# peterdavidfagan/mujoco_robot_environments

Measured on AMD Instinct MI355X. Metric: env steps/sec (whole node), RearrangementEnv batch=4096 at 1/2/4/8 MI355X, higher is better.
Workload: dtype f32

## Files before the change

### mujoco_robot_environments_amd/csrc/mre_dev.h

```cpp
#pragma once
#include <stdint.h>

namespace mre {

constexpr int NB = 20;
constexpr int NRB = 16;
constexpr int GRIP_BODY0 = 8;
constexpr int NV = 39;
constexpr int NRV = 15;
constexpr int NQ = 43;
constexpr int NQP = 44;
constexpr int TRACE_W = 88;
constexpr int TRACE_QVEL = 48;
constexpr int NVP = 40;
constexpr int NU = 8;
constexpr int QFINE = 32;
constexpr int QFINE_ROW = 96;
constexpr int QFINE_CUBE_Q = 32;
constexpr int QFINE_CUBE_V = 60;
static_assert(QFINE_CUBE_Q + 7 * 4 == QFINE_CUBE_V && QFINE_CUBE_V + 6 * 4 <= QFINE_ROW, "qfine row layout");
constexpr int NPROP = 4;
constexpr int NG = 20;
constexpr int PROP_GEOM0 = 12;
constexpr int NPAIR = 128;
// ... 20 lines not shown
constexpr int MAXBLK = 58;
#elif defined(MRE_LARGE_CAPS)
constexpr int NCON_MAX = 44;
constexpr int NEFC_MAX = 148;
constexpr int NRROW_MAX = 83;
constexpr int NPP_MAX = 16;
constexpr int MAXBLK = 52;
#elif defined(MRE_NEWTON)
constexpr int NCON_MAX = 32;
constexpr int NEFC_MAX = 112;
constexpr int NRROW_MAX = 69;
constexpr int NPP_MAX = 8;
constexpr int MAXBLK = 40;
#else
constexpr int NCON_MAX = 32;
constexpr int NEFC_MAX = 112;
constexpr int NRROW_MAX = 62;
constexpr int NPP_MAX = 8;
constexpr int MAXBLK = 40;
#endif
constexpr int NRROW_MAX_COMPACT_PGS = 62, NRROW_MAX_COMPACT_NEWTON = 69;
#if !defined(MRE_LARGE_CAPS)
static_assert(NRROW_MAX ==
#ifdef MRE_NEWTON
              NRROW_MAX_COMPACT_NEWTON,
#else
              NRROW_MAX_COMPACT_PGS,
#endif
              "host-side copy of the compact robot-row capacity");
#endif
static_assert(NEFC_MAX <= 256 && NRROW_MAX < 127 && NPP_MAX <= 16 && MAXBLK >= 8 + NCON_MAX,
              "capacities must fit the block descriptor fields (mre_solver.h)");

struct alignas(16) PairRec {
  int g1, g2, b1, b2;
  int pid1, pid2, type1, single;
  float pos1[3], rb1;
  float pos2[3], rb2;
  float quat1[4], quat2[4];
  float size1[3], margin;
  float size2[3], gap;
};
static_assert(sizeof(PairRec) == 128, "PairRec is eight 16-byte words");

struct alignas(16) BodyRec {
  float quat[4];
  float pos[3], mass;
  float jnt_pos[3], qpos0;
  float jnt_axis[3]; int qposadr;
  float ipos[3]; int propid;
  float iquat[4];
  float inertia[3]; int dofadr;
  float jnt_range[2], invweight0[2];
  float jnt_stiffness, jnt_springref; int parent, jnt_limited;
};
static_assert(sizeof(BodyRec) == 144, "BodyRec is nine 16-byte words");
struct alignas(16) DofRec {
  int body, propid, dofadr, ten;
  float armature, damping, invweight0, ten_coef;
  float jnt_stiffness, jnt_springref, act_gain, act_bias0;
  float act_bias1, act_bias2, act_ctrl_lo, act_ctrl_hi;
  float act_force_lo, act_force_hi; int act_forcelimited, pad;
};
static_assert(sizeof(DofRec) == 80, "DofRec is five 16-byte words");
struct alignas(16) MEntryRec {
  int i, j; float armature, damping;
  float act_bias2, ten_coef; int ten, pad;
};
static_assert(sizeof(MEntryRec) == 32, "MEntryRec is two 16-byte words");
struct alignas(16) RowRec {
  float solref[2], margin, gap;
  float solimp[5], friction;
  float invw1, invw2;
};
static_assert(sizeof(RowRec) == 48, "RowRec is three 16-byte words");
constexpr int ROWREC_JNT = NEQ, ROWREC_PAIR = NEQ + NB, NROWREC = NEQ + NB + NPAIR;
// ... 3 lines not shown
  float data[8];
  float qpos0_1, qpos0_2; int pad2, root_chain_len;
  int root_chain[12];
};
static_assert(sizeof(EqRec) == 128 && MAXCHAIN <= 12, "EqRec is eight 16-byte words");
struct alignas(16) SiteRec {
  float pos[3]; int body;
  float quat[4];
};
static_assert(sizeof(SiteRec) == 32, "SiteRec is two 16-byte words");
struct alignas(16) OptRec {
  float timestep, impratio, tolerance; int iterations;
  float gravity[3]; int cone;
  float ten_coef[2]; int ten_dof[2];
  float grip_gainprm, grip_biasprm[3];
  float grip_forcerange[2], grip_ctrlrange[2];
  float robot_mass, M0_diag_robot_sum; int tcp_site, eef_site;
  float tcp_pos[3]; int pad;
};
static_assert(sizeof(OptRec) == 112, "OptRec is seven 16-byte words");

struct DevModel {
  int body_propid[NB];
  int chain_len[NB];
  int chain_dof[NB][MAXCHAIN];
  float body_mass[NB];
  int dof_Madr[NV + 1];
  float qpos0[NQP];
  int M_i[NMR], M_j[NMR];
  int geom_type[NG], geom_body[NG], geom_propid[NG];
  float geom_size[NG][3], geom_pos[NG][3], geom_quat[NG][4], geom_rbound[NG];
  int pair_g1[NPAIR], pair_g2[NPAIR];
  float pair_margin[NPAIR];
  PairRec pair_rec[NPAIR];
  float act_ctrlrange[NU][2];
  float home_qpos[7];
  float park_pos[NPROP][3];
  BodyRec body_rec[NB];
  DofRec dof_rec[NV];
  MEntryRec m_rec[NMR];
  RowRec row_rec[NROWREC];
  EqRec eq_rec[NEQ];
  SiteRec site_rec[NSITE];
  OptRec opt_rec;
};

struct OscConfig {
  float kp_pos, kd_pos, kp_ori, kd_ori, kp_null, kd_null;
  float null_q[7];
  float pos_thresh, ori_thresh;
  int pinv_always;
};

enum StepFlags : unsigned { F_NO_CONSTRAINTS = 1u, F_FREEZE_ROBOT = 2u, F_CONV_CONTINUE = 4u, F_CONV_OPEN = 8u,
                            F_OSC_EVAL = 16u, F_DETECT = 32u, F_SETTLE_EXIT = 64u, F_DETECT_ACTIVE = 128u,
                            F_CLIP_ALWAYS = 256u, F_NW_ALL_TILES = 512u };
enum CtrlMode : int { CTRL_HELD = 0, CTRL_SEQ = 1, CTRL_OSC = 2 };

struct StepArgs {
  const DevModel* M;
  int N;
  float* qpos;
  float* qvel;
  float* qacc_ws;
  float* qfine;
  float* ctrl;
// ... 127 lines not shown
```

### mujoco_robot_environments_amd/csrc/mre_model.cpp

```cpp
#include "mre_model.h"

#include <cstdint>
#include <cstring>
#include <vector>

#include "../../include/mre.h"

namespace mre {

namespace {
struct Blob {
  const unsigned char* p;
  size_t n;
  bool find(const char* name, uint32_t* code, uint32_t* count, uint64_t* off) const {
    uint32_t ne;
    memcpy(&ne, p + 8, 4);
    const unsigned char* t = p + 16;
    for (uint32_t k = 0; k < ne; k++, t += 48)
      if (strncmp((const char*)t, name, 32) == 0) {
        memcpy(code, t + 32, 4); memcpy(count, t + 36, 4); memcpy(off, t + 40, 8);
        return *off + (size_t)(*count) * (*code ? 8 : 4) <= n;
      }
    return false;
  }
// ... 72 lines not shown
  for (int e = 0; e < NEQ; e++) {
    RowRec& r = m.row_rec[e];
    const int b1 = t.eq_obj[e][0], b2 = t.eq_obj[e][1];
    for (int c = 0; c < 2; c++) r.solref[c] = t.eq_solref[e][c];
    for (int c = 0; c < 5; c++) r.solimp[c] = t.eq_solimp[e][c];
    r.invw1 = e < 2 ? t.body_invweight0[b1][0] : t.dof_invweight0[b1 - 1];
    r.invw2 = e < 2 ? t.body_invweight0[b2][0] : t.dof_invweight0[b2 - 1];
    EqRec& q = m.eq_rec[e];
    memset(&q, 0, sizeof(q));
    q.type = t.eq_type[e]; q.b1 = b1; q.b2 = b2; q.pb1 = t.body_parent[b1]; q.pb2 = t.body_parent[b2];
    q.root = b1;
    while (q.root >= GRIP_BODY0) q.root = t.body_parent[q.root];
    for (int c = 0; c < 8; c++) q.data[c] = t.eq_data[e][c];
    q.qpos0_1 = t.qpos0[b1 - 1]; q.qpos0_2 = t.qpos0[b2 - 1];
    q.root_chain_len = t.chain_len[q.root];
    for (int c = 0; c < MAXCHAIN; c++) q.root_chain[c] = t.chain_dof[q.root][c];
  }
  for (int b = 1; b < NRB; b++) {
    RowRec& r = m.row_rec[ROWREC_JNT + b];
    for (int c = 0; c < 2; c++) r.solref[c] = t.jnt_solref[b][c];
    for (int c = 0; c < 5; c++) r.solimp[c] = t.jnt_solimp[b][c];
    r.invw1 = t.dof_invweight0[b - 1];
  }
  for (int k = 0; k < NPAIR; k++) {
    if (t.pair_g1[k] < 0) continue;
    RowRec& r = m.row_rec[ROWREC_PAIR + k];
    const int b1 = t.geom_body[t.pair_g1[k]], b2 = t.geom_body[t.pair_g2[k]];
    for (int c = 0; c < 2; c++) r.solref[c] = t.pair_solref[k][c];
    for (int c = 0; c < 5; c++) r.solimp[c] = t.pair_solimp[k][c];
    r.margin = t.pair_margin[k]; r.gap = t.pair_gap[k]; r.friction = t.pair_friction[k][0];
    r.invw1 = (b1 > 0 && b1 < NRB) ? t.body_invweight0[b1][0] : 0.f;
    r.invw2 = (b2 > 0 && b2 < NRB) ? t.body_invweight0[b2][0] : 0.f;
  }
  for (int k = 0; k < NSITE; k++) {
    SiteRec& r = m.site_rec[k];
    memset(&r, 0, sizeof(r));
    if (t.site_body[k] < 0 || t.site_body[k] >= NB) return "site_bodyid names a body that does not exist";
    r.body = t.site_body[k];
    for (int c = 0; c < 3; c++) r.pos[c] = t.site_pos[k][c];
    for (int c = 0; c < 4; c++) r.quat[c] = t.site_quat[k][c];
  }
  {
    OptRec& o = m.opt_rec;
    memset(&o, 0, sizeof(o));
    o.timestep = t.timestep; o.impratio = t.impratio; o.tolerance = t.tolerance; o.iterations = t.iterations;
    for (int c = 0; c < 3; c++) { o.gravity[c] = t.gravity[c]; o.grip_biasprm[c] = t.grip_biasprm[c]; }
    o.cone = t.cone;
    for (int c = 0; c < 2; c++) { o.ten_coef[c] = t.ten_coef[c]; o.ten_dof[c] = t.ten_dof[c]; o.grip_forcerange[c] = t.grip_forcerange[c];
                                  o.grip_ctrlrange[c] = t.act_ctrlrange[NU - 1][c]; }
    o.grip_gainprm = t.grip_gainprm; o.robot_mass = t.robot_mass; o.M0_diag_robot_sum = t.M0_diag_robot_sum;
    o.tcp_site = t.tcp_site; o.eef_site = t.eef_site;
    for (int c = 0; c < 3; c++) o.tcp_pos[c] = t.site_pos[t.tcp_site][c];
  }

  bool ok = true;
#define SAME(a, b) ok = ok && sizeof(a) == sizeof(b) && same_bits(&(a), &(b), sizeof(a))
  for (int b = 0; b < NB && ok; b++) {
    const BodyRec& r = m.body_rec[b];
    SAME(r.quat, t.body_quat[b]); SAME(r.pos, t.body_pos[b]); SAME(r.mass, t.body_mass[b]); SAME(r.jnt_pos, t.jnt_pos[b]);
    SAME(r.jnt_axis, t.jnt_axis[b]); SAME(r.qposadr, t.body_qposadr[b]); SAME(r.ipos, t.body_ipos[b]);
    SAME(r.propid, t.body_propid[b]); SAME(r.iquat, t.body_iquat[b]); SAME(r.inertia, t.body_inertia[b]);
    SAME(r.dofadr, t.body_dofadr[b]); SAME(r.jnt_range, t.jnt_range[b]); SAME(r.invweight0, t.body_invweight0[b]);
    SAME(r.jnt_stiffness, t.jnt_stiffness[b]); SAME(r.jnt_springref, t.jnt_springref[b]); SAME(r.parent, t.body_parent[b]);
    SAME(r.jnt_limited, t.jnt_limited[b]);
    if (b >= 1) SAME(r.qpos0, t.qpos0[t.body_qposadr[b]]);
  }
// ... 19 lines not shown
    SAME(r.armature, t.dof_armature[i]); SAME(r.damping, t.dof_damping[i]);
    if (i < 7) SAME(r.act_bias2, t.act_bias[i][2]);
    ok = ok && r.ten == (i == t.ten_dof[0] ? 0 : (i == t.ten_dof[1] ? 1 : -1));
    if (r.ten >= 0) SAME(r.ten_coef, t.ten_coef[r.ten]);
  }
  for (int e = 0; e < NEQ && ok; e++) {
    const RowRec& r = m.row_rec[e];
    const EqRec& q = m.eq_rec[e];
    const int b1 = t.eq_obj[e][0], b2 = t.eq_obj[e][1];
    SAME(r.solref, t.eq_solref[e]); SAME(r.solimp, t.eq_solimp[e]);
    if (e < 2) { SAME(r.invw1, t.body_invweight0[b1][0]); SAME(r.invw2, t.body_invweight0[b2][0]); }
    else { SAME(r.invw1, t.dof_invweight0[b1 - 1]); SAME(r.invw2, t.dof_invweight0[b2 - 1]); }
    SAME(q.type, t.eq_type[e]); SAME(q.b1, t.eq_obj[e][0]); SAME(q.b2, t.eq_obj[e][1]);
    SAME(q.pb1, t.body_parent[b1]); SAME(q.pb2, t.body_parent[b2]); SAME(q.data, t.eq_data[e]);
    SAME(q.qpos0_1, t.qpos0[b1 - 1]); SAME(q.qpos0_2, t.qpos0[b2 - 1]);
    int root = b1;
    while (root >= GRIP_BODY0) root = t.body_parent[root];
    ok = ok && q.root == root;
    SAME(q.root_chain_len, t.chain_len[root]);
    for (int c = 0; c < MAXCHAIN; c++) SAME(q.root_chain[c], t.chain_dof[root][c]);
  }
  for (int b = 1; b < NRB && ok; b++) {
    const RowRec& r = m.row_rec[ROWREC_JNT + b];
    SAME(r.solref, t.jnt_solref[b]); SAME(r.solimp, t.jnt_solimp[b]); SAME(r.invw1, t.dof_invweight0[b - 1]);
  }
  for (int k = 0; k < NPAIR && ok; k++) {
    if (t.pair_g1[k] < 0) continue;
    const RowRec& r = m.row_rec[ROWREC_PAIR + k];
    const int b1 = t.geom_body[t.pair_g1[k]], b2 = t.geom_body[t.pair_g2[k]];
    SAME(r.solref, t.pair_solref[k]); SAME(r.solimp, t.pair_solimp[k]); SAME(r.margin, t.pair_margin[k]);
    SAME(r.gap, t.pair_gap[k]); SAME(r.friction, t.pair_friction[k][0]);
    if (b1 > 0 && b1 < NRB) SAME(r.invw1, t.body_invweight0[b1][0]);
    if (b2 > 0 && b2 < NRB) SAME(r.invw2, t.body_invweight0[b2][0]);
  }
  for (int k = 0; k < NSITE && ok; k++) {
    const SiteRec& r = m.site_rec[k];
    SAME(r.body, t.site_body[k]); SAME(r.pos, t.site_pos[k]); SAME(r.quat, t.site_quat[k]);
  }
  {
    const OptRec& o = m.opt_rec;
    SAME(o.timestep, t.timestep); SAME(o.impratio, t.impratio); SAME(o.tolerance, t.tolerance); SAME(o.iterations, t.iterations);
    SAME(o.gravity, t.gravity); SAME(o.cone, t.cone); SAME(o.ten_coef, t.ten_coef); SAME(o.ten_dof, t.ten_dof);
    SAME(o.grip_gainprm, t.grip_gainprm); SAME(o.grip_biasprm, t.grip_biasprm); SAME(o.grip_forcerange, t.grip_forcerange);
    SAME(o.grip_ctrlrange, t.act_ctrlrange[NU - 1]); SAME(o.robot_mass, t.robot_mass);
    SAME(o.M0_diag_robot_sum, t.M0_diag_robot_sum); SAME(o.tcp_site, t.tcp_site); SAME(o.eef_site, t.eef_site);
    SAME(o.tcp_pos, t.site_pos[t.tcp_site]);
  }
#undef SAME
  if (!ok) return "a packed model record differs from the table it was filled from";
  return std::string();
}

std::string build_model(const void* blob, size_t nbytes, DevModel& m, int& solver) {
  if (nbytes < 16) return "blob too small";
  Blob b{(const unsigned char*)blob, nbytes};
  uint32_t magic;
  memcpy(&magic, b.p, 4);
  if (magic != 0x4D524542u) return "bad blob magic";
  uint32_t nentry;
  memcpy(&nentry, b.p + 8, 4);
  if (16 + 48 * (size_t)nentry > nbytes) return "blob too small";
  ModelTables t;
  memset(&t, 0, sizeof(t));
  memset(&m, 0, sizeof(m));
  int nbody, nv, nq, nM, ngeom, nsite, npair, neq, nprop, nu;
  RI("nbody", &nbody, 1); RI("nv", &nv, 1); RI("nq", &nq, 1); RI("nM", &nM, 1); RI("ngeom", &ngeom, 1);
// ... 1 lines not shown
  RI("nu", &nu, 1);
  if (nbody != NB || nv != NV || nq != NQ || ngeom != NG || nsite != NSITE || npair > NPAIR ||
      neq != NEQ || nprop != NPROP || nu != NU)
    return "scene dimensions differ from the compiled kernels";
  int body_jnttype[NB], act_dof[NU];
  RI("body_parentid", t.body_parent, NB); RI("body_jnttype", body_jnttype, NB);
  RI("body_dofadr", t.body_dofadr, NB); RI("body_qposadr", t.body_qposadr, NB);
  RI("body_propid", t.body_propid, NB);
  RF("body_pos", t.body_pos, NB * 3); RF("body_quat", t.body_quat, NB * 4);
  RF("body_ipos", t.body_ipos, NB * 3); RF("body_iquat", t.body_iquat, NB * 4);
  RF("body_mass", t.body_mass, NB); RF("body_inertia", t.body_inertia, NB * 3);
  RF("body_invweight0", t.body_invweight0, NB * 2);
  RF("jnt_pos", t.jnt_pos, NB * 3); RF("jnt_axis", t.jnt_axis, NB * 3); RF("jnt_range", t.jnt_range, NB * 2);
  RF("jnt_stiffness", t.jnt_stiffness, NB); RF("jnt_springref", t.jnt_springref, NB);
  RF("jnt_solref", t.jnt_solref, NB * 2); RF("jnt_solimp", t.jnt_solimp, NB * 5);
  RI("jnt_limited", t.jnt_limited, NB);
  RI("dof_bodyid", t.dof_body, NV); RI("dof_parentid", t.dof_parent, NV); RI("dof_Madr", t.dof_Madr, NV);
  t.dof_Madr[NV] = nM;
  RF("dof_armature", t.dof_armature, NV); RF("dof_damping", t.dof_damping, NV);
  RF("dof_invweight0", t.dof_invweight0, NV); RF("qpos0", t.qpos0, NQ);
  RI("geom_type", t.geom_type, NG); RI("geom_bodyid", t.geom_body, NG); RI("geom_propid", t.geom_propid, NG);
  RF("geom_size", t.geom_size, NG * 3); RF("geom_pos", t.geom_pos, NG * 3);
  RF("geom_quat", t.geom_quat, NG * 4); RF("geom_rbound", t.geom_rbound, NG);
  {
    std::vector<int> pg(2 * npair);
    RI("pair_geom", pg.data(), 2 * npair);
    for (int k = 0; k < NPAIR; k++) { t.pair_g1[k] = -1; t.pair_g2[k] = -1; }
    for (int k = 0; k < npair; k++) { t.pair_g1[k] = pg[2 * k]; t.pair_g2[k] = pg[2 * k + 1]; }
  }
  RI("pair_single", t.pair_single, npair);
  RF("pair_friction", t.pair_friction, npair * 3); RF("pair_solref", t.pair_solref, npair * 2);
  RF("pair_solimp", t.pair_solimp, npair * 5); RF("pair_margin", t.pair_margin, npair);
  RF("pair_gap", t.pair_gap, npair);
  for (int k = 0; k < NPAIR; k++) {
    PairRec& r = m.pair_rec[k];
    memset(&r, 0, sizeof(r));
    r.g1 = t.pair_g1[k]; r.g2 = t.pair_g2[k];
    if (r.g1 < 0) { r.g2 = -1; r.b1 = r.b2 = 0; r.pid1 = r.pid2 = -1; continue; }
    if (r.g1 >= NG || r.g2 < 0 || r.g2 >= NG) return "pair table names a geom that does not exist";
    r.b1 = t.geom_body[r.g1]; r.b2 = t.geom_body[r.g2];
    r.pid1 = t.geom_propid[r.g1]; r.pid2 = t.geom_propid[r.g2];
    r.type1 = t.geom_type[r.g1]; r.single = (t.pair_single[k] & 0xFF) | (t.geom_type[r.g2] << 8);
    if (t.geom_type[r.g1] == 2 || (t.geom_type[r.g2] == 2 && t.geom_type[r.g1] != 1))
      return "cylinder pairs: only box (geom 1) - cylinder (geom 2) is implemented";
    for (int c = 0; c < 3; c++) { r.pos1[c] = t.geom_pos[r.g1][c]; r.pos2[c] = t.geom_pos[r.g2][c];
                                  r.size1[c] = t.geom_size[r.g1][c]; r.size2[c] = t.geom_size[r.g2][c]; }
    for (int c = 0; c < 4; c++) { r.quat1[c] = t.geom_quat[r.g1][c]; r.quat2[c] = t.geom_quat[r.g2][c]; }
    r.rb1 = t.geom_rbound[r.g1]; r.rb2 = t.geom_rbound[r.g2];
    r.margin = t.pair_margin[k]; r.gap = t.pair_gap[k];
  }
  RI("site_bodyid", t.site_body, NSITE); RF("site_pos", t.site_pos, NSITE * 3);
  RF("site_quat", t.site_quat, NSITE * 4);
  RI("eef_site", &t.eef_site, 1); RI("tcp_site", &t.tcp_site, 1);
  RI("eq_type", t.eq_type, NEQ); RI("eq_obj", t.eq_obj, NEQ * 2); RF("eq_data", t.eq_data, NEQ * 8);
  RF("eq_solref", t.eq_solref, NEQ * 2); RF("eq_solimp", t.eq_solimp, NEQ * 5);
  RI("ten_dof", t.ten_dof, 2); RF("ten_coef", t.ten_coef, 2);
  RI("act_dof", act_dof, NU); RF("act_ctrlrange", t.act_ctrlrange, NU * 2);
  RF("grip_gainprm", &t.grip_gainprm, 1); RF("grip_biasprm", t.grip_biasprm, 3);
  RF("grip_forcerange", t.grip_forcerange, 2);
  for (int a = 0; a < NU; a++) { t.act_gain[a] = 1.f; t.act_forcelimited[a] = 0; }
  { uint32_t c, cnt; uint64_t off;
    if (b.find("act_gainprm", &c, &cnt, &off)) {
      RF("act_gainprm", t.act_gain, NU); RF("act_biasprm", t.act_bias, NU * 3);
      RF("act_forcerange", t.act_forcerange, NU * 2); RI("act_forcelimited", t.act_forcelimited, NU);
    } }
  RF("opt_timestep", &t.timestep, 1); RF("opt_gravity", t.gravity, 3); RF("opt_impratio", &t.impratio, 1);
  RF("opt_tolerance", &t.tolerance, 1); RI("opt_iterations", &t.iterations, 1);
  solver = MRE_SOLVER_PGS;
  { uint32_t c, cnt; uint64_t off; if (b.find("opt_solver", &c, &cnt, &off)) RI("opt_solver", &solver, 1); }
  if (solver != MRE_SOLVER_PGS && solver != MRE_SOLVER_NEWTON) return "opt_solver must be 0 (PGS) or 2 (Newton)";
  { uint32_t c, cnt; uint64_t off; int cone = 1;
    if (b.find("opt_cone", &c, &cnt, &off)) RI("opt_cone", &cone, 1);
    if (cone != 0 && cone != 1) return "opt_cone must be 0 (pyramidal) or 1 (elliptic)";
    t.cone = cone; }
  RF("home_qpos", t.home_qpos, 7);
  float M0d[NV];
  RF("M0_diag", M0d, NV);

  for (int bb = 1; bb < NB; bb++) {
    bool ok = bb < NRB ? (body_jnttype[bb] == 1 && t.body_dofadr[bb] == bb - 1 && t.body_qposadr[bb] == bb - 1 &&
                          t.body_propid[bb] < 0 && t.body_parent[bb] < bb)
                       : (body_jnttype[bb] == 2 && t.body_dofadr[bb] == NRV + 6 * (bb - NRB) &&
// ... 55 lines not shown
```

### mujoco_robot_environments_amd/csrc/mre_solver.h

```cpp
#pragma once

namespace mre {

constexpr int HDR_NONE = 0xFF;
constexpr int BLK_NONE = 0x7F;
constexpr int SCHED_NONE = 0xFF;
constexpr int TAB_OFF = MAXBLK * 5;
constexpr int TAB_ZEROS = 48;
static_assert(TAB_BYTES == 8 * (TAB_OFF + 1) + 4 * TAB_ZEROS, "operand table size");

#ifndef MRE_NEWTON
MRE_DEV void build_schedule(ModelP M, Sm& s);
#endif
MRE_DEV constexpr int cube_pair_bit(int p, int q) {
  const int a = p < q ? p : q, b = p < q ? q : p;
  return a == 0 ? b - 1 : (a == 1 ? b + 1 : 5);
}

MRE_DEV float prop_invM(const Sm& s, int p, int k) {
  return 1.0f / ((k < 3) ? s.prop_mass[p] : s.prop_inertia[p][k - 3]);
}

MRE_DEV void geom_pose(ModelP M, const Sm& s, int g, float* p, float* R, float* size,
                       float* rbound) {
  const int b = M->geom_body[g];
  float tmp[3], q[4];
  m3mulv(tmp, s.xmat[b], M->geom_pos[g]);
  v3add(p, s.xpos[b], tmp);
  qmul(q, s.xquat[b], M->geom_quat[g]);
  q2mat(R, q);
  const int pid = M->geom_propid[g];
  if (pid >= 0) {
    v3copy(size, s.prop_size[pid]);
    *rbound = v3norm(size);
  } else {
    v3copy(size, M->geom_size[g]);
    *rbound = M->geom_rbound[g];
  }
}

MRE_DEV void geom_center(ModelP M, const Sm& s, int g, float* p, float* rbound) {
  const int b = M->geom_body[g];
  float tmp[3];
  m3mulv(tmp, s.xmat[b], M->geom_pos[g]);
  v3add(p, s.xpos[b], tmp);
  const int pid = M->geom_propid[g];
  *rbound = pid >= 0 ? v3norm(s.prop_size[pid]) : M->geom_rbound[g];
}

MRE_PHASE_FN int collide_broad(ModelP M, Sm& s, int l, bool detect) {
  static_assert(offsetof(Sm, hdr) + sizeof(((Sm*)0)->hdr) - offsetof(Sm, JpA) >= sizeof(float) * 64 * COLL_BUF,
                "clip buffers do not fit");
  static_assert(NPAIR <= 256 && sizeof(((Sm*)0)->iscr) >= NPAIR, "survivor list: one byte per pair");
  MRE_DBG_T0();
  uint8_t* list = reinterpret_cast<uint8_t*>(s.iscr);
  const unsigned long long lt = (1ull << l) - 1ull;
  int nsurv = 0;
  for (int pass = 0; pass < NPAIR / 64; pass++) {
    const int pr = l + 64 * pass;
    const auto* R = &M->pair_rec[pr];
    const int g1 = R->g1, b1 = R->b1, b2 = R->b2, pid1 = R->pid1, pid2 = R->pid2, type1 = R->type1;
    const float lp1[3] = {R->pos1[0], R->pos1[1], R->pos1[2]}, lp2[3] = {R->pos2[0], R->pos2[1], R->pos2[2]};
    const float mrb1 = R->rb1, mrb2 = R->rb2, margin = R->margin, gap = R->gap;
    const float lq1[4] = {R->quat1[0], R->quat1[1], R->quat1[2], R->quat1[3]};
    bool live = false;
    if (g1 >= 0 && (pid1 < 0 || pid1 < s.nprops) && (pid2 < 0 || pid2 < s.nprops)) {
      const float inc = detect ? margin : margin - gap;
      float p1[3], p2[3], df[3], tmp[3];
      m3mulv(tmp, s.xmat[b1], lp1); v3add(p1, s.xpos[b1], tmp);
      m3mulv(tmp, s.xmat[b2], lp2); v3add(p2, s.xpos[b2], tmp);
      const float rb1 = pid1 >= 0 ? v3norm(s.prop_size[pid1]) : mrb1, rb2 = pid2 >= 0 ? v3norm(s.prop_size[pid2]) : mrb2;
      v3sub(df, p2, p1);
      if (type1 == 0) {
        float q[4], R1[9];
        qmul(q, s.xquat[b1], lq1);
        q2mat(R1, q);
        const float nn[3] = {R1[2], R1[5], R1[8]};
        live = v3dot(df, nn) - rb2 <= inc;
      } else {
        const float r = rb1 + rb2 + inc;
        live = v3dot(df, df) <= r * r;
      }
    }
    const unsigned long long m = __ballot(live);
    if (live) list[nsurv + __popcll(m & lt)] = (uint8_t)pr;
    nsurv += __popcll(m);
  }
  if (l == 0) s.ncon = 0;
  MRE_SYNC();
  MRE_DBG_STAMP(6, 0);
  return nsurv;
}
MRE_PHASE_FN int collide_narrow(ModelP M, Sm& s, int l, bool detect, bool clip_always, int c0, int nsurv, int base) {
  MRE_DBG_T0();
  float* buf = &s.JpA[0][0] + l * COLL_BUF;
  const uint8_t* list = reinterpret_cast<const uint8_t*>(s.iscr);
  const unsigned long long lt = (1ull << l) - 1ull;
  {
    const int pr = (c0 + l < nsurv) ? list[c0 + l] : -1;
    float normal[3] = {0.f, 0.f, 1.f};
    int n = 0;
    FaceCand rc;
    unsigned rm = 0u;
    if (pr >= 0) {
      const auto* R = &M->pair_rec[pr];
      const int b1 = R->b1, b2 = R->b2, pid1 = R->pid1, pid2 = R->pid2, type1 = R->type1;
      const float lp1[3] = {R->pos1[0], R->pos1[1], R->pos1[2]}, lp2[3] = {R->pos2[0], R->pos2[1], R->pos2[2]};
      const float lq1[4] = {R->quat1[0], R->quat1[1], R->quat1[2], R->quat1[3]};
      const float lq2[4] = {R->quat2[0], R->quat2[1], R->quat2[2], R->quat2[3]};
      const float ms1[3] = {R->size1[0], R->size1[1], R->size1[2]}, ms2[3] = {R->size2[0], R->size2[1], R->size2[2]};
      const float margin = R->margin, gap = R->gap;
      float p1[3], R1[9], s1[3], p2[3], R2[9], s2[3], tmp[3], q[4];
      m3mulv(tmp, s.xmat[b1], lp1); v3add(p1, s.xpos[b1], tmp);
      qmul(q, s.xquat[b1], lq1); q2mat(R1, q);
      m3mulv(tmp, s.xmat[b2], lp2); v3add(p2, s.xpos[b2], tmp);
      qmul(q, s.xquat[b2], lq2); q2mat(R2, q);
      if (pid1 >= 0) v3copy(s1, s.prop_size[pid1]); else v3copy(s1, ms1);
      if (pid2 >= 0) v3copy(s2, s.prop_size[pid2]); else v3copy(s2, ms2);
      const float inc = detect ? margin : margin - gap;
      MRE_DBG_STAMP(6, 1);
      if ((R->single >> 8) == 2) n = cyl_box(p1, R1, s1, p2, R2, s2[0], s2[2], inc, normal, buf);
      else if (type1 == 0) n = plane_box(p1, R1, p2, R2, s2, inc, normal, buf);
      else n = box_box(p1, R1, s1, p2, R2, s2, inc, normal, buf, clip_always, rc, rm);
      MRE_DBG_STAMP(6, 2);
      int m = 0;
      if (rm & FACE_IN_REGS) {
#pragma unroll
        for (int v = 0; v < 4; v++) {
          if (((rm >> v) & 1u) != 0u && rc.d[v] < inc) m++;
          else rm &= ~(1u << v);
        }
      } else {
        for (int c = 0; c < n; c++)
          if (cand_dist(buf, c) < inc) {
            if (m != c) {
              for (int k = 0; k < 3; k++) cand_xyz(buf, m)[k] = cand_xyz(buf, c)[k];
              cand_dist(buf, m) = cand_dist(buf, c);
            }
            m++;
          }
      }
      n = m;
    }
#if defined(MRE_PHASE_STAMPS) && MRE_PHASE_STAMPS == 8
    {
      const bool tbl = pr >= 0 && (M->pair_rec[pr].g1 == 1);
      const unsigned long long fb = __ballot((rm & FACE_BRANCH) != 0u), fr = __ballot((rm & FACE_IN_REGS) != 0u), tb = __ballot(tbl);
      if (l == 0) {
        dbg_acc[0] += (unsigned long long)__popcll(fb) << 4; dbg_acc[1] += (unsigned long long)__popcll(fr) << 4;
        dbg_acc[2] += (unsigned long long)__popcll(fb & tb) << 4; dbg_acc[3] += (unsigned long long)__popcll(fr & tb) << 4;
      }
    }
#endif
    const bool single = pr >= 0 && n > 1 && (M->pair_rec[pr].single & 0xFF) != 0;
    const int ncand = n;
    if (single) n = 1;
    int off = base, tot = base;
    for (int bit = 0; bit < 4; bit++) {
      const unsigned long long m = __ballot((n >> bit) & 1);
      off += __popcll(m & lt) << bit;
      tot += __popcll(m) << bit;
    }
    if (l == 0) {
      s.ncon = tot < NCON_MAX ? tot : NCON_MAX;
      if (tot > NCON_MAX) s.overflow = 1;
    }
    if (single) {
      const float incw = M->pair_rec[pr].margin - M->pair_rec[pr].gap;
      if (rm & FACE_IN_REGS) {
        float wsum = 0.f, px = 0.f, py = 0.f, pz = 0.f, dmin = 0.f, bx = 0.f, by = 0.f, bz = 0.f;
        bool first = true;
#pragma unroll
        for (int v = 0; v < 4; v++)
          if (((rm >> v) & 1u) != 0u) {
            const float dc = rc.d[v];
            if (first || dc < dmin) { dmin = dc; bx = rc.x[v]; by = rc.y[v]; bz = rc.z[v]; }
            first = false;
            const float w = incw - dc;
            if (w > 0.f) { wsum += w; px += w * rc.x[v]; py += w * rc.y[v]; pz += w * rc.z[v]; }
          }
        if (wsum > 0.f) { const float iw = 1.0f / wsum; px *= iw; py *= iw; pz *= iw; }
        else { px = bx; py = by; pz = bz; }
        rc.x[0] = px; rc.y[0] = py; rc.z[0] = pz; rc.d[0] = dmin;
        rm = FACE_IN_REGS | 1u;
      } else {
        float wsum = 0.f, px = 0.f, py = 0.f, pz = 0.f, dmin = cand_dist(buf, 0);
        int best = 0;
        for (int c = 0; c < ncand; c++) {
          const float dc = cand_dist(buf, c);
          if (dc < dmin) { dmin = dc; best = c; }
          const float w = incw - dc;
          if (w > 0.f) { wsum += w; px += w * cand_xyz(buf, c)[0]; py += w * cand_xyz(buf, c)[1]; pz += w * cand_xyz(buf, c)[2]; }
        }
        if (wsum > 0.f) { const float iw = 1.0f / wsum; px *= iw; py *= iw; pz *= iw; }
        else { px = cand_xyz(buf, best)[0]; py = cand_xyz(buf, best)[1]; pz = cand_xyz(buf, best)[2]; }
        cand_xyz(buf, 0)[0] = px; cand_xyz(buf, 0)[1] = py; cand_xyz(buf, 0)[2] = pz;
        cand_dist(buf, 0) = dmin;
      }
    }
    if (n > 0) {
      float f[9];
      v3copy(f, normal);
      make_frame(f);
      if (rm & FACE_IN_REGS) {
        int id = off;
#pragma unroll
        for (int v = 0; v < 4; v++)
          if (((rm >> v) & 1u) != 0u && id < NCON_MAX) {
            s.con_pos[id][0] = rc.x[v]; s.con_pos[id][1] = rc.y[v]; s.con_pos[id][2] = rc.z[v];
            for (int k = 0; k < 9; k++) s.con_frame[id][k] = f[k];
            s.con_dist[id] = rc.d[v];
            s.con_pair[id] = (uint8_t)pr;
            id++;
          }
      } else {
        for (int c = 0; c < n; c++) {
          const int id = off + c;
          if (id >= NCON_MAX) break;
          const float cx0 = cand_xyz(buf, c)[0], cx1 = cand_xyz(buf, c)[1], cx2 = cand_xyz(buf, c)[2];
          s.con_pos[id][0] = cx0; s.con_pos[id][1] = cx1; s.con_pos[id][2] = cx2;
          for (int k = 0; k < 9; k++) s.con_frame[id][k] = f[k];
          s.con_dist[id] = cand_dist(buf, c);
          s.con_pair[id] = (uint8_t)pr;
        }
      }
    }
    MRE_SYNC();
    MRE_DBG_STAMP(6, 3);
    return tot;
  }
}
MRE_DEV void collide(ModelP M, Sm& s, int l, bool detect, bool clip_always) {
  const int nsurv = collide_broad(M, s, l, detect);
  int base = 0;
  for (int c0 = 0; c0 < nsurv; c0 += 64) {
    base = collide_narrow(M, s, l, detect, clip_always, c0, nsurv, base);
    if (base > NCON_MAX) break;
  }
}

MRE_DEV float impedance(const float* solimp, float pos, float margin) {
  const float dmin = clampf(solimp[0], 0.0001f, 0.9999f), dmax = clampf(solimp[1], 0.0001f, 0.9999f);
  const float width = fmaxf(solimp[2], kMinVal), mid = clampf(solimp[3], 0.0001f, 0.9999f);
  const float power = fmaxf(solimp[4], 1.0f);
  if (dmin == dmax) return 0.5f * (dmin + dmax);
  const float x = fabsf((pos - margin) / width);
  if (x >= 1.0f) return dmax;
  if (x <= 0.0f) return dmin;
  float y;
  if (power == 1.0f) y = x;
  else if (power == 2.0f) {
    y = (x <= mid) ? x * x / mid : 1.0f - (1.0f - x) * (1.0f - x) / (1.0f - mid);
  }
  else if (x <= mid) y = powf(x, power) / powf(mid, power - 1.0f);
  else y = 1.0f - powf(1.0f - x, power) / powf(1.0f - mid, power - 1.0f);
  return dmin + y * (dmax - dmin);
}

MRE_DEV void jac_robot(ModelP M, Sm& s, int rs, int b, const float* p, const float* ax, float sg) {
  float off[3];
  v3sub(off, p, s.com_robot);
  const int n = M->chain_len[b];
  for (int k = 0; k < n; k++) {
    const int j = M->chain_dof[b][k];
    const float* c = s.cdof[j];
    float t[3];
// ... 65 lines not shown

#ifndef MRE_NEWTON
MRE_PHASE_FN void solve_robot_rows(Sm& s, int l) {
  for (int rs = l; rs < s.nrrow; rs += 64) {
    float x[NRV];
#pragma unroll
    for (int k = 0; k < NRV; k++) x[k] = s.Jr[rs][k];
    solve_robot_regs(s.qLD, s.qLDinv, x);
#pragma unroll
    for (int k = 0; k < NRV; k++) s.Br[rs][k] = x[k];
  }
  MRE_SYNC();
}

#endif

constexpr int GRIP0 = GRIP_BODY0;

MRE_PHASE_FN void assemble_constraints(ModelP M, Sm& s, int l) {
  int lim = 0, lim_side = 0;
  const auto* BR = &M->body_rec[l < NRB ? l : 0];
  const int jnt_limited = BR->jnt_limited;
  const float jnt_range[2] = {BR->jnt_range[0], BR->jnt_range[1]};
  if (l >= 1 && l < NRB && jnt_limited) {
    const double q = robot_q(s, l - 1);
    if (q - (double)jnt_range[0] < 0.0) { lim = 1; lim_side = -1; }
    else if ((double)jnt_range[1] - q < 0.0) { lim = 1; lim_side = 1; }
  }
  keep_live(jnt_range[0]); keep_live(jnt_range[1]);
  const unsigned long long limm = __ballot(lim != 0);
  const int lim_idx = __popcll(limm & ((1ull << l) - 1ull));
  if (l == 0) s.nl = __popcll(limm);
  if (lim) s.lim_info[lim_idx] = l | ((lim_side > 0 ? 1 : 0) << 8);
  if (l < s.ncon) {
    const int pr = s.con_pair[l];
    s.con_b1[l] = (uint8_t)M->pair_rec[pr].b1;
    s.con_b2[l] = (uint8_t)M->pair_rec[pr].b2;
  }
  MRE_SYNC();
#ifndef MRE_NEWTON
  {
    static_assert(sizeof(s.sched) % 4 == 0, "schedule cleared by words");
    unsigned* w = reinterpret_cast<unsigned*>(&s.sched[0][0]);
    for (int e = l; e < (int)(sizeof(s.sched) / 4); e += 64) w[e] = 0x01010101u * (unsigned)SCHED_NONE;
  }
#endif
  {
    const int base = 7 + s.nl, ncon0 = s.ncon;
    const bool on = l < ncon0;
    const int cb1 = on ? s.con_b1[l] : 0, cb2 = on ? s.con_b2[l] : 0;
    const bool rob_any = on && ((cb1 < NRB && cb1 > 0) || (cb2 < NRB && cb2 > 0));
    const bool fing = on && ((cb1 >= GRIP_BODY0 && cb1 < NRB) || (cb2 >= GRIP_BODY0 && cb2 < NRB));
    const unsigned long long fingm = __ballot(fing);
    const bool two_props = on && cb1 >= NRB && cb2 >= NRB;
    const unsigned long long lt = (1ull << l) - 1ull;
    const unsigned long long rmask = __ballot(rob_any), tmask = __ballot(two_props);
    const int my_r = base + 3 * __popcll(rmask & lt), my_b = __popcll(tmask & lt);
    const bool fail = on && (base + 3 * (l + 1) > NEFC_MAX || (rob_any && my_r + 3 > NRROW_MAX) ||
                             (two_props && my_b >= NPP_MAX));
    const unsigned long long fmask = __ballot(fail);
    const int kept = fmask != 0ull ? (int)__builtin_ctzll(fmask) : ncon0;
    if (l < kept) {
      s.con_rslot[l] = rob_any ? my_r : HDR_NONE;
      s.con_bslot[l] = two_props ? my_b : 0;
    }
    MRE_SYNC();
    if (l == 0) {
      const unsigned long long below = kept >= 64 ? ~0ull : ((1ull << kept) - 1ull);
      if (fmask != 0ull) s.overflow = 1;
      s.ncon = kept;
      s.nefc = base + 3 * kept;
// ... 705 lines not shown
```

Measured before the change: 25.92 million.

## Precompute per-geom world frames in shared memory and pack pair records

Adds a per-geom pass in which each lane computes one geom's world position, rotation matrix, size and bounding radius into a shared-memory table placed behind the clip buffers. Broad and narrow phase then read that table instead of redoing the transform and quaternion-to-matrix work per pair. PairRec shrinks from 128 to 16 bytes by bit-packing indices, and contact body ids are written during narrow phase rather than looked up in assemble_constraints. The cost is an extra barrier and reuse of scratch shared memory, guarded by static asserts, plus a debug counter for survivor counts.

```diff
diff --git a/mujoco_robot_environments_amd/csrc/mre_dev.h b/mujoco_robot_environments_amd/csrc/mre_dev.h
--- a/mujoco_robot_environments_amd/csrc/mre_dev.h
+++ b/mujoco_robot_environments_amd/csrc/mre_dev.h
@@ -76,16 +76,32 @@
 static_assert(NEFC_MAX <= 256 && NRROW_MAX < 127 && NPP_MAX <= 16 && MAXBLK >= 8 + NCON_MAX,
               "capacities must fit the block descriptor fields (mre_solver.h)");
 
+struct alignas(16) GeomRec {
+  int body, propid, type; float rbound;
+  float pos[3]; int pad0;
+  float quat[4];
+  float size[3]; int pad1;
+};
+static_assert(sizeof(GeomRec) == 64, "GeomRec is four 16-byte words");
 struct alignas(16) PairRec {
-  int g1, g2, b1, b2;
-  int pid1, pid2, type1, single;
-  float pos1[3], rb1;
-  float pos2[3], rb2;
-  float quat1[4], quat2[4];
-  float size1[3], margin;
-  float size2[3], gap;
-};
-static_assert(sizeof(PairRec) == 128, "PairRec is eight 16-byte words");
+  uint32_t geoms;
+  uint32_t kinds;
+  float margin, gap;
+};
+struct PairK { int g1, g2, b1, b2, pid1, pid2, type1, type2, single; float margin, gap; };
+constexpr uint32_t pair_geoms_word(int g1, int g2, int b1, int b2) {
+  return g1 < 0 ? 0xFFFFu : (uint32_t)g1 | (uint32_t)g2 << 8 | (uint32_t)b1 << 16 | (uint32_t)b2 << 24;
+}
+constexpr uint32_t pair_kinds_word(int pid1, int pid2, int type1, int type2, int single) {
+  return (uint32_t)(pid1 + 1) | (uint32_t)(pid2 + 1) << 8 | (uint32_t)type1 << 16 | (uint32_t)type2 << 20 | (uint32_t)single << 24;
+}
+constexpr PairK pair_unpack(uint32_t geoms, uint32_t kinds, float margin, float gap) {
+  return PairK{(geoms & 0xFF) == 0xFF ? -1 : (int)(geoms & 0xFF), (geoms & 0xFF) == 0xFF ? -1 : (int)((geoms >> 8) & 0xFF),
+               (int)((geoms >> 16) & 0xFF), (int)(geoms >> 24), (int)(kinds & 0xFF) - 1, (int)((kinds >> 8) & 0xFF) - 1,
+               (int)((kinds >> 16) & 0xF), (int)((kinds >> 20) & 0xF), (int)(kinds >> 24), margin, gap};
+}
+static_assert(sizeof(PairRec) == 16 && NG < 255 && NB <= 256 && NPROP < 255, "PairRec is one 16-byte word");
+constexpr int GEOM_TAB_W = 16;
 
 struct alignas(16) BodyRec {
   float quat[4];
@@ -155,6 +171,7 @@
   float geom_size[NG][3], geom_pos[NG][3], geom_quat[NG][4], geom_rbound[NG];
   int pair_g1[NPAIR], pair_g2[NPAIR];
   float pair_margin[NPAIR];
+  GeomRec geom_rec[NG];
   PairRec pair_rec[NPAIR];
   float act_ctrlrange[NU][2];
   float home_qpos[7];
diff --git a/mujoco_robot_environments_amd/csrc/mre_model.cpp b/mujoco_robot_environments_amd/csrc/mre_model.cpp
--- a/mujoco_robot_environments_amd/csrc/mre_model.cpp
+++ b/mujoco_robot_environments_amd/csrc/mre_model.cpp
@@ -128,6 +128,22 @@
     r.invw1 = (b1 > 0 && b1 < NRB) ? t.body_invweight0[b1][0] : 0.f;
     r.invw2 = (b2 > 0 && b2 < NRB) ? t.body_invweight0[b2][0] : 0.f;
   }
+  for (int g = 0; g < NG; g++) {
+    GeomRec& r = m.geom_rec[g];
+    memset(&r, 0, sizeof(r));
+    r.body = t.geom_body[g]; r.propid = t.geom_propid[g]; r.type = t.geom_type[g]; r.rbound = t.geom_rbound[g];
+    for (int c = 0; c < 3; c++) { r.pos[c] = t.geom_pos[g][c]; r.size[c] = t.geom_size[g][c]; }
+    for (int c = 0; c < 4; c++) r.quat[c] = t.geom_quat[g][c];
+  }
+  for (int k = 0; k < NPAIR; k++) {
+    PairRec& r = m.pair_rec[k];
+    memset(&r, 0, sizeof(r));
+    const int g1 = t.pair_g1[k], g2 = t.pair_g2[k];
+    if (g1 < 0) { r.geoms = pair_geoms_word(-1, -1, 0, 0); continue; }
+    r.geoms = pair_geoms_word(g1, g2, t.geom_body[g1], t.geom_body[g2]);
+    r.kinds = pair_kinds_word(t.geom_propid[g1], t.geom_propid[g2], t.geom_type[g1], t.geom_type[g2], t.pair_single[k] & 0xFF);
+    r.margin = t.pair_margin[k]; r.gap = t.pair_gap[k];
+  }
   for (int k = 0; k < NSITE; k++) {
     SiteRec& r = m.site_rec[k];
     memset(&r, 0, sizeof(r));
@@ -213,6 +229,21 @@
     SAME(r.gap, t.pair_gap[k]); SAME(r.friction, t.pair_friction[k][0]);
     if (b1 > 0 && b1 < NRB) SAME(r.invw1, t.body_invweight0[b1][0]);
     if (b2 > 0 && b2 < NRB) SAME(r.invw2, t.body_invweight0[b2][0]);
+  }
+  for (int g = 0; g < NG && ok; g++) {
+    const GeomRec& r = m.geom_rec[g];
+    SAME(r.body, t.geom_body[g]); SAME(r.propid, t.geom_propid[g]); SAME(r.type, t.geom_type[g]);
+    SAME(r.rbound, t.geom_rbound[g]); SAME(r.pos, t.geom_pos[g]); SAME(r.quat, t.geom_quat[g]); SAME(r.size, t.geom_size[g]);
+  }
+  for (int k = 0; k < NPAIR && ok; k++) {
+    const PairRec& r = m.pair_rec[k];
+    const PairK p = pair_unpack(r.geoms, r.kinds, r.margin, r.gap);
+    if (t.pair_g1[k] < 0) { ok = ok && p.g1 < 0; continue; }
+    const int g1 = t.pair_g1[k], g2 = t.pair_g2[k];
+    ok = ok && p.g1 == g1 && p.g2 == g2 && p.b1 == t.geom_body[g1] && p.b2 == t.geom_body[g2] &&
+         p.pid1 == t.geom_propid[g1] && p.pid2 == t.geom_propid[g2] && p.type1 == t.geom_type[g1] &&
+         p.type2 == t.geom_type[g2] && p.single == (t.pair_single[k] & 0xFF);
+    SAME(r.margin, t.pair_margin[k]); SAME(r.gap, t.pair_gap[k]);
   }
   for (int k = 0; k < NSITE && ok; k++) {
     const SiteRec& r = m.site_rec[k];
@@ -280,22 +311,17 @@
   RF("pair_friction", t.pair_friction, npair * 3); RF("pair_solref", t.pair_solref, npair * 2);
   RF("pair_solimp", t.pair_solimp, npair * 5); RF("pair_margin", t.pair_margin, npair);
   RF("pair_gap", t.pair_gap, npair);
+  for (int g = 0; g < NG; g++) {
+    if (t.geom_body[g] < 0 || t.geom_body[g] >= NB) return "geom_bodyid names a body that does not exist";
+    if (t.geom_propid[g] < -1 || t.geom_propid[g] >= NPROP) return "geom_propid names a cube slot that does not exist";
+    if (t.geom_type[g] < 0 || t.geom_type[g] > 15) return "geom_type is none the kernels know";
+  }
   for (int k = 0; k < NPAIR; k++) {
-    PairRec& r = m.pair_rec[k];
-    memset(&r, 0, sizeof(r));
-    r.g1 = t.pair_g1[k]; r.g2 = t.pair_g2[k];
-    if (r.g1 < 0) { r.g2 = -1; r.b1 = r.b2 = 0; r.pid1 = r.pid2 = -1; continue; }
-    if (r.g1 >= NG || r.g2 < 0 || r.g2 >= NG) return "pair table names a geom that does not exist";
-    r.b1 = t.geom_body[r.g1]; r.b2 = t.geom_body[r.g2];
-    r.pid1 = t.geom_propid[r.g1]; r.pid2 = t.geom_propid[r.g2];
-    r.type1 = t.geom_type[r.g1]; r.single = (t.pair_single[k] & 0xFF) | (t.geom_type[r.g2] << 8);
-    if (t.geom_type[r.g1] == 2 || (t.geom_type[r.g2] == 2 && t.geom_type[r.g1] != 1))
+    const int g1 = t.pair_g1[k], g2 = t.pair_g2[k];
+    if (g1 < 0) continue;
+    if (g1 >= NG || g2 < 0 || g2 >= NG) return "pair table names a geom that does not exist";
+    if (t.geom_type[g1] == 2 || (t.geom_type[g2] == 2 && t.geom_type[g1] != 1))
       return "cylinder pairs: only box (geom 1) - cylinder (geom 2) is implemented";
-    for (int c = 0; c < 3; c++) { r.pos1[c] = t.geom_pos[r.g1][c]; r.pos2[c] = t.geom_pos[r.g2][c];
-                                  r.size1[c] = t.geom_size[r.g1][c]; r.size2[c] = t.geom_size[r.g2][c]; }
-    for (int c = 0; c < 4; c++) { r.quat1[c] = t.geom_quat[r.g1][c]; r.quat2[c] = t.geom_quat[r.g2][c]; }
-    r.rb1 = t.geom_rbound[r.g1]; r.rb2 = t.geom_rbound[r.g2];
-    r.margin = t.pair_margin[k]; r.gap = t.pair_gap[k];
   }
   RI("site_bodyid", t.site_body, NSITE); RF("site_pos", t.site_pos, NSITE * 3);
   RF("site_quat", t.site_quat, NSITE * 4);
diff --git a/mujoco_robot_environments_amd/csrc/mre_solver.h b/mujoco_robot_environments_amd/csrc/mre_solver.h
--- a/mujoco_robot_environments_amd/csrc/mre_solver.h
+++ b/mujoco_robot_environments_amd/csrc/mre_solver.h
@@ -39,43 +39,67 @@
   }
 }
 
-MRE_DEV void geom_center(ModelP M, const Sm& s, int g, float* p, float* rbound) {
-  const int b = M->geom_body[g];
-  float tmp[3];
-  m3mulv(tmp, s.xmat[b], M->geom_pos[g]);
-  v3add(p, s.xpos[b], tmp);
-  const int pid = M->geom_propid[g];
-  *rbound = pid >= 0 ? v3norm(s.prop_size[pid]) : M->geom_rbound[g];
+MRE_DEV float* geom_tab(Sm& s) { return &s.JpA[0][0] + 64 * COLL_BUF; }
+MRE_DEV PairK load_pair(ModelP M, int pr) {
+  const auto* R = &M->pair_rec[pr];
+  return pair_unpack(R->geoms, R->kinds, R->margin, R->gap);
 }
 
 MRE_PHASE_FN int collide_broad(ModelP M, Sm& s, int l, bool detect) {
   static_assert(offsetof(Sm, hdr) + sizeof(((Sm*)0)->hdr) - offsetof(Sm, JpA) >= sizeof(float) * 64 * COLL_BUF,
                 "clip buffers do not fit");
   static_assert(NPAIR <= 256 && sizeof(((Sm*)0)->iscr) >= NPAIR, "survivor list: one byte per pair");
+  static_assert(offsetof(Sm, hdr) + sizeof(((Sm*)0)->hdr) - offsetof(Sm, JpA) >= sizeof(float) * (64 * COLL_BUF + NG * GEOM_TAB_W),
+                "the geom table does not fit behind the clip buffers");
+#ifdef MRE_NEWTON
+  static_assert(offsetof(Sm, zrow) - offsetof(Sm, JpA) >= sizeof(float) * (64 * COLL_BUF + NG * GEOM_TAB_W),
+                "the geom table would overwrite zrow, which is written once per launch");
+#endif
+  static_assert(NG <= 64, "geom pass: one lane per geom");
   MRE_DBG_T0();
   uint8_t* list = reinterpret_cast<uint8_t*>(s.iscr);
   const unsigned long long lt = (1ull << l) - 1ull;
+  const auto* G = &M->geom_rec[l < NG ? l : 0];
+  const int gb = G->body, gpid = G->propid;
+  const float grb = G->rbound;
+  const float gp[3] = {G->pos[0], G->pos[1], G->pos[2]}, gq[4] = {G->quat[0], G->quat[1], G->quat[2], G->quat[3]};
+  const float gs[3] = {G->size[0], G->size[1], G->size[2]};
+  PairK PK[NPAIR / 64];
+#pragma unroll
+  for (int pass = 0; pass < NPAIR / 64; pass++) PK[pass] = load_pair(M, l + 64 * pass);
+  float* tab = geom_tab(s);
+  if (l < NG) {
+    float p[3], R[9], tmp[3], q[4], size[3], rb;
+    m3mulv(tmp, s.xmat[gb], gp); v3add(p, s.xpos[gb], tmp);
+    qmul(q, s.xquat[gb], gq); q2mat(R, q);
+    if (gpid >= 0) { v3copy(size, s.prop_size[gpid]); rb = v3norm(s.prop_size[gpid]); }
+    else { v3copy(size, gs); rb = grb; }
+    float* o = tab + GEOM_TAB_W * l;
+    for (int k = 0; k < 3; k++) o[k] = p[k];
+    for (int k = 0; k < 9; k++) o[3 + k] = R[k];
+    for (int k = 0; k < 3; k++) o[12 + k] = size[k];
+    o[15] = rb;
+  }
+  keep_live(gs[0]); keep_live(gs[1]); keep_live(gs[2]); keep_live(grb);
+  MRE_SYNC();
   int nsurv = 0;
+#pragma unroll
   for (int pass = 0; pass < NPAIR / 64; pass++) {
     const int pr = l + 64 * pass;
-    const auto* R = &M->pair_rec[pr];
-    const int g1 = R->g1, b1 = R->b1, b2 = R->b2, pid1 = R->pid1, pid2 = R->pid2, type1 = R->type1;
-    const float lp1[3] = {R->pos1[0], R->pos1[1], R->pos1[2]}, lp2[3] = {R->pos2[0], R->pos2[1], R->pos2[2]};
-    const float mrb1 = R->rb1, mrb2 = R->rb2, margin = R->margin, gap = R->gap;
-    const float lq1[4] = {R->quat1[0], R->quat1[1], R->quat1[2], R->quat1[3]};
+    const PairK P = PK[pass];
+    const int g1 = P.g1, g2 = P.g2, pid1 = P.pid1, pid2 = P.pid2, type1 = P.type1;
+    const float margin = P.margin, gap = P.gap;
     bool live = false;
     if (g1 >= 0 && (pid1 < 0 || pid1 < s.nprops) && (pid2 < 0 || pid2 < s.nprops)) {
       const float inc = detect ? margin : margin - gap;
-      float p1[3], p2[3], df[3], tmp[3];
-      m3mulv(tmp, s.xmat[b1], lp1); v3add(p1, s.xpos[b1], tmp);
-      m3mulv(tmp, s.xmat[b2], lp2); v3add(p2, s.xpos[b2], tmp);
-      const float rb1 = pid1 >= 0 ? v3norm(s.prop_size[pid1]) : mrb1, rb2 = pid2 >= 0 ? v3norm(s.prop_size[pid2]) : mrb2;
+      const float* A = tab + GEOM_TAB_W * g1;
+      const float* B = tab + GEOM_TAB_W * g2;
+      const float p1[3] = {A[0], A[1], A[2]}, p2[3] = {B[0], B[1], B[2]};
+      const float rb1 = A[15], rb2 = B[15];
+      float df[3];
       v3sub(df, p2, p1);
       if (type1 == 0) {
-        float q[4], R1[9];
-        qmul(q, s.xquat[b1], lq1);
-        q2mat(R1, q);
-        const float nn[3] = {R1[2], R1[5], R1[8]};
+        const float nn[3] = {A[3 + 2], A[3 + 5], A[3 + 8]};
         live = v3dot(df, nn) - rb2 <= inc;
       } else {
         const float r = rb1 + rb2 + inc;
@@ -102,24 +126,18 @@
     int n = 0;
     FaceCand rc;
     unsigned rm = 0u;
+    const PairK P = load_pair(M, pr >= 0 ? pr : 0);
     if (pr >= 0) {
-      const auto* R = &M->pair_rec[pr];
-      const int b1 = R->b1, b2 = R->b2, pid1 = R->pid1, pid2 = R->pid2, type1 = R->type1;
-      const float lp1[3] = {R->pos1[0], R->pos1[1], R->pos1[2]}, lp2[3] = {R->pos2[0], R->pos2[1], R->pos2[2]};
-      const float lq1[4] = {R->quat1[0], R->quat1[1], R->quat1[2], R->quat1[3]};
-      const float lq2[4] = {R->quat2[0], R->quat2[1], R->quat2[2], R->quat2[3]};
-      const float ms1[3] = {R->size1[0], R->size1[1], R->size1[2]}, ms2[3] = {R->size2[0], R->size2[1], R->size2[2]};
-      const float margin = R->margin, gap = R->gap;
-      float p1[3], R1[9], s1[3], p2[3], R2[9], s2[3], tmp[3], q[4];
-      m3mulv(tmp, s.xmat[b1], lp1); v3add(p1, s.xpos[b1], tmp);
-      qmul(q, s.xquat[b1], lq1); q2mat(R1, q);
-      m3mulv(tmp, s.xmat[b2], lp2); v3add(p2, s.xpos[b2], tmp);
-      qmul(q, s.xquat[b2], lq2); q2mat(R2, q);
-      if (pid1 >= 0) v3copy(s1, s.prop_size[pid1]); else v3copy(s1, ms1);
-      if (pid2 >= 0) v3copy(s2, s.prop_size[pid2]); else v3copy(s2, ms2);
+      const int type1 = P.type1;
+      const float margin = P.margin, gap = P.gap;
+      const float* A = geom_tab(s) + GEOM_TAB_W * P.g1;
+      const float* B = geom_tab(s) + GEOM_TAB_W * P.g2;
+      float p1[3], R1[9], s1[3], p2[3], R2[9], s2[3];
+      for (int k = 0; k < 3; k++) { p1[k] = A[k]; s1[k] = A[12 + k]; p2[k] = B[k]; s2[k] = B[12 + k]; }
+      for (int k = 0; k < 9; k++) { R1[k] = A[3 + k]; R2[k] = B[3 + k]; }
       const float inc = detect ? margin : margin - gap;
       MRE_DBG_STAMP(6, 1);
-      if ((R->single >> 8) == 2) n = cyl_box(p1, R1, s1, p2, R2, s2[0], s2[2], inc, normal, buf);
+      if (P.type2 == 2) n = cyl_box(p1, R1, s1, p2, R2, s2[0], s2[2], inc, normal, buf);
       else if (type1 == 0) n = plane_box(p1, R1, p2, R2, s2, inc, normal, buf);
       else n = box_box(p1, R1, s1, p2, R2, s2, inc, normal, buf, clip_always, rc, rm);
       MRE_DBG_STAMP(6, 2);
@@ -144,7 +162,7 @@
     }
 #if defined(MRE_PHASE_STAMPS) && MRE_PHASE_STAMPS == 8
     {
-      const bool tbl = pr >= 0 && (M->pair_rec[pr].g1 == 1);
+      const bool tbl = pr >= 0 && P.g1 == 1;
       const unsigned long long fb = __ballot((rm & FACE_BRANCH) != 0u), fr = __ballot((rm & FACE_IN_REGS) != 0u), tb = __ballot(tbl);
       if (l == 0) {
         dbg_acc[0] += (unsigned long long)__popcll(fb) << 4; dbg_acc[1] += (unsigned long long)__popcll(fr) << 4;
@@ -152,7 +170,7 @@
       }
     }
 #endif
-    const bool single = pr >= 0 && n > 1 && (M->pair_rec[pr].single & 0xFF) != 0;
+    const bool single = pr >= 0 && n > 1 && P.single != 0;
     const int ncand = n;
     if (single) n = 1;
     int off = base, tot = base;
@@ -166,7 +184,7 @@
       if (tot > NCON_MAX) s.overflow = 1;
     }
     if (single) {
-      const float incw = M->pair_rec[pr].margin - M->pair_rec[pr].gap;
+      const float incw = P.margin - P.gap;
       if (rm & FACE_IN_REGS) {
         float wsum = 0.f, px = 0.f, py = 0.f, pz = 0.f, dmin = 0.f, bx = 0.f, by = 0.f, bz = 0.f;
         bool first = true;
@@ -210,7 +228,7 @@
             s.con_pos[id][0] = rc.x[v]; s.con_pos[id][1] = rc.y[v]; s.con_pos[id][2] = rc.z[v];
             for (int k = 0; k < 9; k++) s.con_frame[id][k] = f[k];
             s.con_dist[id] = rc.d[v];
-            s.con_pair[id] = (uint8_t)pr;
+            s.con_pair[id] = (uint8_t)pr; s.con_b1[id] = (uint8_t)P.b1; s.con_b2[id] = (uint8_t)P.b2;
             id++;
           }
       } else {
@@ -221,7 +239,7 @@
           s.con_pos[id][0] = cx0; s.con_pos[id][1] = cx1; s.con_pos[id][2] = cx2;
           for (int k = 0; k < 9; k++) s.con_frame[id][k] = f[k];
           s.con_dist[id] = cand_dist(buf, c);
-          s.con_pair[id] = (uint8_t)pr;
+          s.con_pair[id] = (uint8_t)pr; s.con_b1[id] = (uint8_t)P.b1; s.con_b2[id] = (uint8_t)P.b2;
         }
       }
     }
@@ -232,6 +250,12 @@
 }
 MRE_DEV void collide(ModelP M, Sm& s, int l, bool detect, bool clip_always) {
   const int nsurv = collide_broad(M, s, l, detect);
+#if defined(MRE_PHASE_STAMPS) && MRE_PHASE_STAMPS == 12
+  if (l == 0) {
+    dbg_acc[0] += (unsigned long long)nsurv << 4; dbg_acc[1] += (unsigned long long)(nsurv > 16) << 4;
+    dbg_acc[2] += (unsigned long long)(nsurv > 32) << 4; dbg_acc[3] += (unsigned long long)(nsurv > 64) << 4;
+  }
+#endif
   int base = 0;
   for (int c0 = 0; c0 < nsurv; c0 += 64) {
     base = collide_narrow(M, s, l, detect, clip_always, c0, nsurv, base);
@@ -363,11 +387,6 @@
   const int lim_idx = __popcll(limm & ((1ull << l) - 1ull));
   if (l == 0) s.nl = __popcll(limm);
   if (lim) s.lim_info[lim_idx] = l | ((lim_side > 0 ? 1 : 0) << 8);
-  if (l < s.ncon) {
-    const int pr = s.con_pair[l];
-    s.con_b1[l] = (uint8_t)M->pair_rec[pr].b1;
-    s.con_b2[l] = (uint8_t)M->pair_rec[pr].b2;
-  }
   MRE_SYNC();
 #ifndef MRE_NEWTON
   {
```

Result: no change. 26.12 million (median of 6 runs) (+0.8%).
